# ToKe79/nuts333

Hardware: AMD Instinct MI355X
Metric: delivered_broadcast_lines_per_s (higher is better)
Workload: dtype u8

## Files before the change

nuts333_amd/device/fanout.hip:

```cpp

#include <hip/hip_runtime.h>
#include <hipcub/hipcub.hpp>

#include <algorithm>
#include <chrono>
#include <cstdint>
#include <cstdio>
#include <cstring>

namespace {

constexpr int kOutBuff = 1000;
constexpr int kTextSize = 2000;
constexpr int kNumCols = 21;
constexpr int kMaxWrites = 16;
constexpr int kBlock = 256;

constexpr uint8_t kLogin = 1, kHasRoom = 2, kSameRoom = 4, kIgnall = 8, kIgnshout = 16, kSender = 32, kColour = 64;
constexpr int kComShout = 4, kComSemote = 7;

__constant__ char kColCom[kNumCols][2] = {
    {'R', 'S'}, {'O', 'L'}, {'U', 'L'}, {'L', 'I'}, {'R', 'V'}, {'F', 'K'}, {'F', 'R'}, {'F', 'G'}, {'F', 'Y'}, {'F', 'B'},
    {'F', 'M'}, {'F', 'T'}, {'F', 'W'}, {'B', 'K'}, {'B', 'R'}, {'B', 'G'}, {'B', 'Y'}, {'B', 'B'}, {'B', 'M'}, {'B', 'T'},
    {'B', 'W'},
};
__constant__ char kColArg[kNumCols][2] = {
    {'0', 0}, {'1', 0}, {'4', 0}, {'5', 0}, {'7', 0}, {'3', '0'}, {'3', '1'}, {'3', '2'}, {'3', '3'}, {'3', '4'},
    {'3', '5'}, {'3', '6'}, {'3', '7'}, {'4', '0'}, {'4', '1'}, {'4', '2'}, {'4', '3'}, {'4', '4'}, {'4', '5'}, {'4', '6'},
    {'4', '7'},
};

__device__ __forceinline__ bool admits(uint8_t l, int rm_is_null, int force_listen, int com_num)
{
    if (l & kLogin) return false;
    if (!(l & kHasRoom)) return false;
    if (!(l & kSameRoom) && !rm_is_null) return false;
    if ((l & kIgnall) && !force_listen) return false;
    if ((l & kIgnshout) && (com_num == kComShout || com_num == kComSemote)) return false;
    if (l & kSender) return false;
    return true;
}

__device__ __forceinline__ uint8_t listener_record(int room, uint8_t slot, int rm, int sender, int j)
{
    return (slot & (kLogin | kIgnall | kIgnshout | kColour)) | (room >= 0 ? kHasRoom : 0) |
           (rm >= 0 && room == rm ? kSameRoom : 0) | (j == sender ? kSender : 0);
}

__device__ __forceinline__ int colcom_at(const uint8_t* s, int i, int len)
{
    if (i + 2 >= len) return -1;
    const uint8_t a = s[i + 1], b = s[i + 2];
    for (int c = 0; c < kNumCols; c++)
        if (a == (uint8_t)kColCom[c][0] && b == (uint8_t)kColCom[c][1]) return c;
    return -1;
}

template <bool EMIT>
struct Sink {
    uint8_t* out;
    int32_t* wsz;
    int64_t cap;
    int wcap;
    int64_t n = 0;
    int writes = 0;
    int pos = 0;

    __device__ __forceinline__ void put(uint8_t c)
    {
        if (EMIT && n < cap) out[n] = c;
        n++;
        pos++;
    }
    __device__ __forceinline__ void flush()
    {
        if (EMIT && writes < wcap) wsz[writes] = pos;
        writes++;
        pos = 0;
    }
    __device__ __forceinline__ void reset_code()
    {
        put(27); put('['); put('0'); put('m');
    }
};

template <bool EMIT>
__device__ void transduce(const uint8_t* s, int len, bool colour, Sink<EMIT>& k)
{
    int i = 0;
    while (i < len) {
        const uint8_t ch = s[i];
        if (ch == '\n') {
            if (k.pos > kOutBuff - 6) k.flush();
            if (colour) k.reset_code();
            k.put('\n');
            k.put('\r');
            i++;
        } else if (ch == '/' && i + 1 < len && s[i + 1] == '~') {
            i++;
            continue;
        } else if (i > 0 && ch == '~' && s[i - 1] == '/') {
            k.put('~');
            i++;
        } else if (ch == '~') {
            if (k.pos > kOutBuff - 6) k.flush();
            const int c = colcom_at(s, i, len);
            if (c >= 0) {
                if (colour) {
                    k.put(27); k.put('['); k.put((uint8_t)kColArg[c][0]);
                    if (kColArg[c][1]) k.put((uint8_t)kColArg[c][1]);
                    k.put('m');
                }
                i += 3;
            } else {
                k.put('~');
                i++;
            }
        } else {
            k.put(ch);
            i++;
        }
        if (k.pos == kOutBuff) k.flush();
    }
    if (k.pos) k.flush();
    if (colour) {
        k.reset_code();
        k.flush();
    }
}

struct Args {
    const uint8_t* text;
    const int32_t* text_off;
    const int32_t* text_len;
    const uint8_t* rec;
    int n;
    int rm_is_null, force_listen, com_num;
    uint8_t* admitted;
    int64_t* nbytes;
    int32_t* nwrites;
    int64_t* out_off;
    int32_t* w_off;
    int* violations;
    uint8_t* arena;
    int64_t arena_cap;
    int32_t* wsz;
    int64_t wsz_cap;
};

template <bool BROADCAST>
__device__ __forceinline__ bool load_item(const Args& a, int i, const uint8_t*& s, int& len)
{
    if (BROADCAST) {
        __shared__ uint8_t lds[kTextSize];
        len = a.text_len[0];
        for (int j = threadIdx.x; j < len; j += blockDim.x) lds[j] = a.text[j];
        __syncthreads();
        s = lds;
        return i < a.n;
    }
    if (i >= a.n) return false;
    s = a.text + a.text_off[i];
    len = a.text_len[i];
    return true;
}

template <bool BROADCAST>
__device__ void measure(const Args& a)
{
    const int i = blockIdx.x * blockDim.x + threadIdx.x;
    if (i == 0) {
        a.nbytes[a.n] = 0;
        a.nwrites[a.n] = 0;
    }
    const uint8_t* s;
    int len;
    if (!load_item<BROADCAST>(a, i, s, len)) return;
    const uint8_t l = a.rec[i];
    const bool in = !BROADCAST || admits(l, a.rm_is_null, a.force_listen, a.com_num);
    Sink<false> k{nullptr, nullptr, 0, 0};
    if (in) transduce(s, len, (l & kColour) != 0, k);
    if (k.n > 6 * (int64_t)len + 4 || k.writes > kMaxWrites) atomicAdd(a.violations, 1);
    a.admitted[i] = in;
    a.nbytes[i] = k.n;
    a.nwrites[i] = k.writes;
}

template <bool BROADCAST>
__device__ void emit(const Args& a)
{
    const int i = blockIdx.x * blockDim.x + threadIdx.x;
    const uint8_t* s;
    int len;
    if (!load_item<BROADCAST>(a, i, s, len) || !a.admitted[i]) return;
    const int64_t room = a.arena_cap - a.out_off[i], wroom = a.wsz_cap - a.w_off[i];
    const int64_t cap = a.nbytes[i] < room ? a.nbytes[i] : (room > 0 ? room : 0);
    const int wcap = (int)(a.nwrites[i] < wroom ? a.nwrites[i] : (wroom > 0 ? wroom : 0));
    Sink<true> k{a.arena + a.out_off[i], a.wsz + a.w_off[i], cap, wcap};
    transduce(s, len, (a.rec[i] & kColour) != 0, k);
}

constexpr int kVarCap = 6 * (kTextSize - 1) + 4;
constexpr int kGroup = 16;

struct ManyArgs {
    const uint8_t* text;
    const int32_t* text_off;
    const int32_t* text_len;
    const uint8_t* flags;
    const int32_t* com_num;
    const int32_t* item_off;
    const int32_t* tile_off;
    const uint8_t* rec;
    int k, m;
    int* violations;
    uint8_t* admitted;
    int64_t* out_off;
    int32_t* w_off;
    int64_t* nbytes;
    int32_t* nwrites;
    uint8_t* arena;
    int64_t arena_cap;
    int32_t* wsz;
    int64_t wsz_cap;
};

struct Tile {
    int b, lo, hi;
};

__device__ __forceinline__ Tile find_tile(const ManyArgs& a)
{
    const int blk = (int)blockIdx.x;
    int lo = 0, hi = a.k;
    while (hi - lo > 1) {
        const int mid = (lo + hi) >> 1;
        if (a.tile_off[mid] <= blk) lo = mid;
        else hi = mid;
    }
    const int first = a.item_off[lo] + (blk - a.tile_off[lo]) * kBlock;
    const int end = a.item_off[lo + 1];
    return {lo, first, first + kBlock < end ? first + kBlock : end};
}

template <bool EMIT, typename A>
__device__ __forceinline__ void stage_variants(const A& a, int b, uint8_t* text, uint8_t* var, int32_t* vwsz,
                                               int64_t* vn, int* vw)
{
    const int len = a.text_len[b];
    const uint8_t* src = a.text + a.text_off[b];
    for (int j = threadIdx.x; j < len; j += blockDim.x) text[j] = src[j];
    __syncthreads();
    if (threadIdx.x == 0 || threadIdx.x == 64) {
        const int c = threadIdx.x >> 6;
        Sink<EMIT> k{EMIT ? var + c * kVarCap : nullptr, EMIT ? vwsz + c * kMaxWrites : nullptr, 6 * (int64_t)len + 4,
                     kMaxWrites};
        transduce(text, len, c != 0, k);
        vn[c] = k.n;
        vw[c] = k.writes;
    }
    __syncthreads();
}

__device__ void measure_many(const ManyArgs& a)
{
    __shared__ uint8_t text[kTextSize];
    __shared__ int64_t vn[2];
    __shared__ int vw[2];
    if (blockIdx.x == 0 && threadIdx.x == 0) {
        a.nbytes[a.m] = 0;
        a.nwrites[a.m] = 0;
    }
    const Tile t = find_tile(a);
    stage_variants<false>(a, t.b, text, nullptr, nullptr, vn, vw);
    const int i = t.lo + (int)threadIdx.x;
    if (i >= t.hi) return;
    const uint8_t l = a.rec[i];
    const int fl = a.flags[t.b];
    const bool in = admits(l, fl & 1, (fl >> 1) & 1, a.com_num[t.b]);
    const int c = (l & kColour) ? 1 : 0;
    const int64_t nb = in ? vn[c] : 0;
    const int nw = in ? vw[c] : 0;
    if (nb > 6 * (int64_t)a.text_len[t.b] + 4 || nw > kMaxWrites) atomicAdd(a.violations, 1);
    a.admitted[i] = in;
    a.nbytes[i] = nb;
    a.nwrites[i] = nw;
}

__device__ void emit_many(const ManyArgs& a)
{
    __shared__ uint8_t text[kTextSize];
    __shared__ uint8_t var[2 * kVarCap];
    __shared__ int32_t vwsz[2 * kMaxWrites];
    __shared__ int64_t vn[2];
    __shared__ int vw[2];
    __shared__ int64_t s_off[kBlock], s_n[kBlock];
    __shared__ int32_t s_woff[kBlock], s_nw[kBlock];
    __shared__ uint8_t s_c[kBlock];
    const Tile t = find_tile(a);
    const int len = a.text_len[t.b];
    {
        const int i = t.lo + (int)threadIdx.x;
        if (i < t.hi) {
            const bool in = a.admitted[i] != 0;
            const int64_t off = a.out_off[i], woff = a.w_off[i];
            const int64_t room = a.arena_cap - off, wroom = a.wsz_cap - woff;
            int64_t n = in ? a.nbytes[i] : 0;
            n = n < room ? n : room;
            n = n < 6 * (int64_t)len + 4 ? n : 6 * (int64_t)len + 4;
            int64_t nw = in ? a.nwrites[i] : 0;
            nw = nw < wroom ? nw : wroom;
            nw = nw < kMaxWrites ? nw : kMaxWrites;
            s_off[threadIdx.x] = off;
            s_n[threadIdx.x] = n > 0 ? n : 0;
            s_woff[threadIdx.x] = (int32_t)woff;
            s_nw[threadIdx.x] = nw > 0 ? (int32_t)nw : 0;
            s_c[threadIdx.x] = (a.rec[i] & kColour) ? 1 : 0;
        }
    }
    stage_variants<true>(a, t.b, text, var, vwsz, vn, vw);
    const int g = (int)threadIdx.x / kGroup, lane = (int)threadIdx.x % kGroup;
    for (int j = g; j < t.hi - t.lo; j += kBlock / kGroup) {
        const int c = s_c[j];
        const int64_t n0 = s_n[j], vmax = vn[c] < kVarCap ? vn[c] : kVarCap;
        const int64_t n = n0 < vmax ? n0 : vmax;
        const uint8_t* src = var + c * kVarCap;
        uint8_t* dst = a.arena + s_off[j];
        const int head = (int)(s_off[j] & 3);
        for (int64_t w = 4 * lane - head; w < n; w += 4 * kGroup) {
            if (w >= 0 && w + 4 <= n) {
                const uint32_t v = (uint32_t)src[w] | (uint32_t)src[w + 1] << 8 | (uint32_t)src[w + 2] << 16 |
                                   (uint32_t)src[w + 3] << 24;
                *reinterpret_cast<uint32_t*>(dst + w) = v;
            } else {
                for (int q = 0; q < 4; q++)
                    if (w + q >= 0 && w + q < n) dst[w + q] = src[w + q];
            }
        }
        const int nw = s_nw[j] < vw[c] ? s_nw[j] : vw[c];
        if (lane < nw) a.wsz[s_woff[j] + lane] = vwsz[c * kMaxWrites + lane];
    }
}

static_assert(kGroup >= kMaxWrites, "emit_many writes an item's chunk sizes with one lane each");
static_assert(kBlock % kGroup == 0 && kBlock >= 128, "emit_many: whole lane groups; variants on waves 0 and 1");

struct RosterArgs {
    const int32_t* room;
    const uint8_t* slot;
    const uint8_t* text;
    const int32_t* text_off;
    const int32_t* text_len;
    const int32_t* rm;
    const int32_t* sender;
    const uint8_t* flags;
    const int32_t* com_num;
    int k, capacity, tiles;
    int* violations;
    uint8_t* admitted;
    int64_t* out_off;
    int32_t* w_off;
    uint8_t* var;
    int64_t* vn;
    int32_t* vw;
    int32_t* vwsz;
    uint8_t* arena;
    int64_t arena_cap;
    int32_t* wsz;
    int64_t wsz_cap;
};

__host__ __device__ __forceinline__ int64_t var_stride(int len) { return (6 * (int64_t)len + 4 + 3) & ~(int64_t)3; }
__host__ __device__ __forceinline__ int64_t var_at(int64_t text_off, int64_t t) { return 12 * text_off + 16 * t; }

template <typename A>
__device__ __forceinline__ void store_variants(const A& a, int t)
{
    __shared__ uint8_t text[kTextSize];
    __shared__ uint8_t var[2 * kVarCap];
    __shared__ int32_t vwsz[2 * kMaxWrites];
    __shared__ int64_t vn[2];
    __shared__ int vw[2];
    stage_variants<true>(a, t, text, var, vwsz, vn, vw);
    const int len = a.text_len[t];
    const int64_t cap = 6 * (int64_t)len + 4, stride = var_stride(len);
    uint8_t* dst = a.var + var_at(a.text_off[t], t);
    for (int c = 0; c < 2; c++) {
        const int64_t n = vn[c] < cap ? vn[c] : cap;
        for (int64_t q = threadIdx.x; q < n; q += kBlock) dst[c * stride + q] = var[c * kVarCap + q];
        const int nw = vw[c] < kMaxWrites ? vw[c] : kMaxWrites;
        if ((int)threadIdx.x < nw) a.vwsz[(2 * t + c) * kMaxWrites + threadIdx.x] = vwsz[c * kMaxWrites + threadIdx.x];
    }
    if (threadIdx.x < 2) {
        a.vn[2 * t + threadIdx.x] = vn[threadIdx.x];
        a.vw[2 * t + threadIdx.x] = vw[threadIdx.x];
        if (vn[threadIdx.x] > cap || vw[threadIdx.x] > kMaxWrites) atomicAdd(a.violations, 1);
    }
}

__device__ void roster_measure(const RosterArgs& a)
{
    const int b = (int)blockIdx.x / a.tiles, tile = (int)blockIdx.x - b * a.tiles;
    const int j = tile * kBlock + (int)threadIdx.x;
    if (j < a.capacity) {
        const int rm = a.rm[b];
        const uint8_t l = listener_record(a.room[j], a.slot[j], rm, a.sender[b], j);
        a.admitted[b * a.capacity + j] = admits(l, rm < 0, (a.flags[b] >> 1) & 1, a.com_num[b]);
    }
    if (tile == 0) store_variants(a, b);
}

template <typename T>
struct ItemCount {
    const uint8_t* admitted;
    const uint8_t* slot;
    const T* v;
    int capacity, m;
    __host__ __device__ T operator()(int i) const
    {
        if (i >= m || !admitted[i]) return 0;
        const int b = i / capacity;
        return v[2 * b + ((slot[i - b * capacity] & kColour) ? 1 : 0)];
    }
};

__device__ __forceinline__ void copy_items(int count, const uint8_t* var, const int32_t* vwsz, const int64_t* vn,
                                           const int* vw, const int64_t* s_off, const int64_t* s_n,
                                           const int32_t* s_woff, const int32_t* s_nw, const uint8_t* s_c,
                                           uint8_t* arena, int32_t* wsz)
{
    const int g = (int)threadIdx.x / kGroup, lane = (int)threadIdx.x % kGroup;
    for (int j = g; j < count; j += kBlock / kGroup) {
        const int c = s_c[j];
        const int64_t n0 = s_n[j], vmax = vn[c] < kVarCap ? vn[c] : kVarCap;
        const int64_t n = n0 < vmax ? n0 : vmax;
        const uint8_t* src = var + c * kVarCap;
        uint8_t* dst = arena + s_off[j];
        const int head = (int)(s_off[j] & 3);
        for (int64_t w = 4 * lane - head; w < n; w += 4 * kGroup) {
            if (w >= 0 && w + 4 <= n) {
                const uint32_t v = (uint32_t)src[w] | (uint32_t)src[w + 1] << 8 | (uint32_t)src[w + 2] << 16 |
                                   (uint32_t)src[w + 3] << 24;
                *reinterpret_cast<uint32_t*>(dst + w) = v;
            } else {
                for (int q = 0; q < 4; q++)
                    if (w + q >= 0 && w + q < n) dst[w + q] = src[w + q];
            }
        }
        const int nw = s_nw[j] < vw[c] ? s_nw[j] : vw[c];
        if (lane < nw) wsz[s_woff[j] + lane] = vwsz[c * kMaxWrites + lane];
    }
}

__device__ void roster_emit(const RosterArgs& a)
{
    __shared__ uint8_t var[2 * kVarCap];
    __shared__ int32_t vwsz[2 * kMaxWrites];
    __shared__ int64_t vn[2];
    __shared__ int vw[2];
    __shared__ int64_t s_off[kBlock], s_n[kBlock];
    __shared__ int32_t s_woff[kBlock], s_nw[kBlock];
    __shared__ uint8_t s_c[kBlock];
    const int b = (int)blockIdx.x / a.tiles, j0 = ((int)blockIdx.x - b * a.tiles) * kBlock;
    const int len = a.text_len[b];
    const int64_t cap = 6 * (int64_t)len + 4;
    {
        const int j = j0 + (int)threadIdx.x;
        if (j < a.capacity) {
            const int i = b * a.capacity + j;
            const bool in = a.admitted[i] != 0;
            const int64_t off = a.out_off[i], woff = a.w_off[i];
            const int64_t room = a.arena_cap - off, wroom = a.wsz_cap - woff;
            int64_t n = in ? a.out_off[i + 1] - off : 0;
            n = n < room ? n : room;
            n = n < cap ? n : cap;
            int64_t nw = in ? a.w_off[i + 1] - woff : 0;
            nw = nw < wroom ? nw : wroom;
            nw = nw < kMaxWrites ? nw : kMaxWrites;
            s_off[threadIdx.x] = off;
            s_n[threadIdx.x] = n > 0 ? n : 0;
            s_woff[threadIdx.x] = (int32_t)woff;
            s_nw[threadIdx.x] = nw > 0 ? (int32_t)nw : 0;
            s_c[threadIdx.x] = (a.slot[j] & kColour) ? 1 : 0;
        }
    }
    const uint8_t* src = a.var + var_at(a.text_off[b], b);
    const int64_t stride = var_stride(len);
    for (int c = 0; c < 2; c++) {
        const int64_t n = a.vn[2 * b + c] < cap ? a.vn[2 * b + c] : cap;
        for (int64_t q = threadIdx.x; q < n; q += kBlock) var[c * kVarCap + q] = src[c * stride + q];
        const int nw = a.vw[2 * b + c] < kMaxWrites ? a.vw[2 * b + c] : kMaxWrites;
        if ((int)threadIdx.x < nw) vwsz[c * kMaxWrites + threadIdx.x] = a.vwsz[(2 * b + c) * kMaxWrites + threadIdx.x];
        if (threadIdx.x == 0) {
            vn[c] = n;
            vw[c] = nw;
        }
    }
    __syncthreads();
    const int count = a.capacity - j0 < kBlock ? a.capacity - j0 : kBlock;
    copy_items(count, var, vwsz, vn, vw, s_off, s_n, s_woff, s_nw, s_c, a.arena, a.wsz);
}

static_assert(2 * kMaxWrites <= kBlock, "roster kernels move a broadcast's chunk sizes with one lane each");

struct PlanArgs {
    const int32_t* room;
    const uint8_t* slot;
    const uint8_t* text;
    const int32_t* text_off;
    const int32_t* text_len;
    const int32_t* rm;
    const int32_t* sender;
    const uint8_t* flags;
    const int32_t* com_num;
    int k, capacity, tiles;
    int words;
    int* violations;
    int64_t* vn;
    int32_t* vw;
    int32_t* vwsz;
    uint64_t* bits;
    uint8_t* var;
};

__device__ void roster_plan(const PlanArgs& a)
{
    const int b = (int)blockIdx.x / a.tiles, tile = (int)blockIdx.x - b * a.tiles;
    const int j = tile * kBlock + (int)threadIdx.x;
    bool in = false;
    if (j < a.capacity) {
        const int rm = a.rm[b];
        const uint8_t l = listener_record(a.room[j], a.slot[j], rm, a.sender[b], j);
        in = admits(l, rm < 0, (a.flags[b] >> 1) & 1, a.com_num[b]);
    }
    const uint64_t word = __ballot(in);
    const int w = j >> 6;
    if ((threadIdx.x & 63) == 0 && w < a.words) a.bits[(int64_t)b * a.words + w] = word;
    if (tile == 0) store_variants(a, b);
}

static_assert(kBlock % 64 == 0, "roster_plan: a tile is whole bitmap words, one per wave");

constexpr int kRevLines = 15;
constexpr int kRevLen = 200;
constexpr int kRevSlot = kRevLen + 2;
constexpr int kRevRing = kRevLines * kRevSlot;
constexpr int kRevLineCap = 6 * (kRevLen + 1) + 4;
constexpr int kRevLineStride = (kRevLineCap + 1 + 3) & ~3;
constexpr int kRevLineWrites = 3;
constexpr int kRevVarCap = kRevLines * kRevLineCap;
constexpr int rev_var_stride(int lines) { return (lines * kRevLineCap + 3) & ~3; }
constexpr int kRevVarStride = rev_var_stride(kRevLines);
constexpr int kTellLines = 5;
constexpr int kRevWrites = kRevLines * kRevLineWrites;
constexpr int kRevTasks = 2 * kRevLines;
constexpr int kWaveLimit = kOutBuff - 6;
constexpr uint8_t kRecordBit = 4;
constexpr int kMaxReviewRooms = 1024;

struct RecordArgs {
    const uint8_t* text;
    const int32_t* text_off;
    const int32_t* text_len;
    const int32_t* rm;
    const uint8_t* flags;
    const uint8_t* clear;
    int k, review_rooms;
    uint8_t* rings;
    int32_t* revline;
};

template <int LINES>
__device__ void roster_record(const RecordArgs& a)
{
    __shared__ int s_surv[LINES];
    __shared__ int s_count, s_base;
    const int room = (int)blockIdx.x;
    const bool cleared = a.clear && a.clear[room];
    if (threadIdx.x < 64) {
        const int lane = (int)threadIdx.x;
        int count = 0;
        for (int b0 = 0; b0 < a.k; b0 += 64) {
            const int b = b0 + lane;
            const bool hit = b < a.k && (a.flags[b] & kRecordBit) && a.rm[b] == room;
            const uint64_t word = __ballot(hit);
            const int n = __popcll(word);
            const int rank = count + __popcll(word & ((1ull << lane) - 1));
            if (hit && rank >= count + n - LINES) s_surv[rank % LINES] = b;
            count += n;
        }
        if (lane == 0) {
            s_count = count;
            s_base = cleared ? 0 : (int)((uint32_t)a.revline[room] % LINES);
        }
    }
    __syncthreads();
    const int count = s_count, base = s_base;
    if (!count && !cleared) return;
    uint8_t* ring = a.rings + (size_t)room * LINES * kRevSlot;
    const int nsurv = count < LINES ? count : LINES;
    const int first = (count - nsurv) % LINES;
    if (cleared && threadIdx.x < LINES) {
        const int d = ((int)threadIdx.x - base - first + 2 * LINES) % LINES;
        if (d >= nsurv) ring[threadIdx.x * kRevSlot] = 0;
    }
    for (int idx = (int)threadIdx.x; idx < nsurv * kRevSlot; idx += kBlock) {
        const int j = idx / kRevSlot, i = idx - j * kRevSlot;
        const int r = (first + j) % LINES;
        const int b = s_surv[r];
        uint8_t v = 0;
        if (i < kRevLen) {
            if (i < a.text_len[b]) v = a.text[a.text_off[b] + i];
        } else if (i == kRevLen) {
            v = '\n';
        }
        ring[((base + r) % LINES) * kRevSlot + i] = v;
    }
    if (threadIdx.x == 0) a.revline[room] = (base + count % LINES) % LINES;
}

struct ReviewArgs {
    uint8_t* rings;
    int32_t* revline;
    const int32_t* rooms;
    const uint8_t* clear;
    int q, review_rooms;
    int* violations;
    int32_t* line_count;
    int32_t* sequential;
    int32_t* vn;
    int32_t* vw;
    int32_t* vwsz;
    uint8_t* lines;
    uint8_t* var;
};

__device__ __forceinline__ int expand_byte(uint8_t p1, uint8_t ch, uint8_t n1, bool consumed, int own, bool colour,
                                           uint64_t* v)
{
    *v = ch;
    if (ch == 0 || consumed) return 0;
    if (ch == '\n') {
        if (colour) {
            *v = 27ull | (uint64_t)'[' << 8 | (uint64_t)'0' << 16 | (uint64_t)'m' << 24 | (uint64_t)'\n' << 32 |
                 (uint64_t)'\r' << 40;
            return 6;
        }
        *v = (uint64_t)'\n' | (uint64_t)'\r' << 8;
        return 2;
    }
    if (ch == '/' && n1 == '~') return 0;
    if (ch == '~' && p1 != '/' && own >= 0) {
        if (!colour) return 0;
        const uint64_t a0 = (uint8_t)kColArg[own][0], a1 = (uint8_t)kColArg[own][1];
        *v = 27ull | (uint64_t)'[' << 8 | a0 << 16 | (a1 ? a1 << 24 | (uint64_t)'m' << 32 : (uint64_t)'m' << 24);
        return a1 ? 5 : 4;
    }
    return 1;
}

template <int LINES>
__device__ void roster_review(const ReviewArgs& a)
{
    constexpr int TASKS = 2 * LINES;
    constexpr int RING = LINES * kRevSlot, WRITES = LINES * kRevLineWrites;
    if ((int)blockIdx.x >= a.q) {
        const int room = ((int)blockIdx.x - a.q) * kBlock + (int)threadIdx.x;
        if (a.clear && room < a.review_rooms && a.clear[room]) {
            for (int i = 0; i < LINES; i++) a.rings[(size_t)room * RING + i * kRevSlot] = 0;
            a.revline[room] = 0;
        }
        return;
    }
    __shared__ uint8_t s_line[LINES][kRevSlot + 2];
    __shared__ uint8_t s_out[TASKS][kRevLineStride];
    __shared__ int32_t s_wsz[TASKS][kRevLineWrites + 1];
    __shared__ int s_n[TASKS], s_w[TASKS], s_off[TASKS], s_woff[TASKS];
    __shared__ int s_len[LINES], s_seq;
    const int q = (int)blockIdx.x, room = a.rooms[q];
    const bool cleared = a.clear && a.clear[room];
    const int rev = cleared ? 0 : (int)((uint32_t)a.revline[room] % LINES);
    const uint8_t* ring = a.rings + (size_t)room * RING;
    for (int idx = (int)threadIdx.x; idx < RING; idx += kBlock) {
        const int i = idx / kRevSlot, j = idx - i * kRevSlot;
        const uint8_t v = cleared ? 0 : ring[((rev + i) % LINES) * kRevSlot + j];
        s_line[i][j] = v;
        a.lines[(size_t)q * RING + idx] = v;
    }
    if (threadIdx.x == 0) s_seq = 0;
    __syncthreads();

    const int lane = (int)threadIdx.x & 63;
    for (int t = (int)threadIdx.x >> 6; t < TASKS; t += kBlock / 64) {
        const int i = t >> 1;
        const bool colour = (t & 1) != 0;
        const uint8_t* s = s_line[i];
        uint8_t w[9];
#pragma unroll
        for (int x = 0; x < 9; x++) {
            const int at = 4 * lane - 3 + x;
            w[x] = at >= 0 && at < kRevSlot ? s[at] : 0;
        }
        const int nul = w[3] == 0 ? 0 : w[4] == 0 ? 1 : w[5] == 0 ? 2 : w[6] == 0 ? 3 : 4;
        const uint64_t ends = __ballot(nul < 4);
        const int end_lane = __ffsll((unsigned long long)ends) - 1;
        const int len = 4 * end_lane + __shfl(nul, end_lane, 64);
#pragma unroll
        for (int x = 0; x < 9; x++)
            if (4 * lane - 3 + x >= len) w[x] = 0;
        int cmd[6], key[6];
        bool tilde = false;
#pragma unroll
        for (int x = 0; x < 6; x++) {
            cmd[x] = -1;
            key[x] = w[x + 1] == '~' && w[x] != '/' ? w[x + 2] << 8 | w[x + 3] : -1;
            tilde |= key[x] >= 0;
        }
        if (tilde) {
#pragma unroll 1
            for (int c = 0; c < kNumCols; c++) {
                const int pair = (uint8_t)kColCom[c][0] << 8 | (uint8_t)kColCom[c][1];
#pragma unroll
                for (int x = 0; x < 6; x++) cmd[x] = key[x] == pair ? c : cmd[x];
            }
        }
        int n[4], mine = 0;
        uint64_t v[4];
#pragma unroll
        for (int x = 0; x < 4; x++) {
            n[x] = expand_byte(w[x + 2], w[x + 3], w[x + 4], cmd[x] >= 0 || cmd[x + 1] >= 0, cmd[x + 2], colour, &v[x]);
            mine += n[x];
        }
        int incl = mine;
#pragma unroll
        for (int d = 1; d < 64; d <<= 1) {
            const int y = __shfl_up(incl, d, 64);
            if (lane >= d) incl += y;
        }
        const int body = __shfl(incl, 63, 64);
        uint8_t* out = s_out[t];
        if (len == 0) {
            if (lane == 0) {
                s_n[t] = 0;
                s_w[t] = 0;
            }
        } else if (body <= kWaveLimit) {
            int at = incl - mine;
#pragma unroll
            for (int x = 0; x < 4; x++) {
#pragma unroll
                for (int y = 0; y < 6; y++)
                    out[y < n[x] ? at + y : kRevLineStride - 1] = (uint8_t)(v[x] >> (8 * y));
                at += n[x];
            }
            if (colour && lane < 4) out[body + lane] = lane == 0 ? 27 : lane == 1 ? '[' : lane == 2 ? '0' : 'm';
            if (lane == 0) {
                int nw = 0;
                if (body) s_wsz[t][nw++] = body;
                if (colour) s_wsz[t][nw++] = 4;
                s_n[t] = body + (colour ? 4 : 0);
                s_w[t] = nw;
            }
        } else if (lane == 0) {
            s_n[t] = -1;
        }
        if (lane == 0 && !colour) s_len[i] = len;
    }
    __syncthreads();
    if (threadIdx.x < TASKS && s_n[threadIdx.x] < 0) {
        const int t = (int)threadIdx.x;
        Sink<true> k{s_out[t], s_wsz[t], kRevLineCap, kRevLineWrites};
        transduce(s_line[t >> 1], s_len[t >> 1], (t & 1) != 0, k);
        if (k.n > kRevLineCap || k.writes > kRevLineWrites) atomicAdd(a.violations, 1);
        s_n[t] = k.n < kRevLineCap ? (int)k.n : kRevLineCap;
        s_w[t] = k.writes < kRevLineWrites ? k.writes : kRevLineWrites;
        atomicAdd(&s_seq, 1);
    }
    __syncthreads();
    if (threadIdx.x < TASKS) {
        const int t = (int)threadIdx.x;
        int off = 0, woff = 0;
        for (int j = t & 1; j < t; j += 2) {
            off += s_n[j];
            woff += s_w[j];
        }
        s_off[t] = off;
        s_woff[t] = woff;
        if (t >= TASKS - 2) {
            a.vn[2 * q + (t & 1)] = off + s_n[t];
            a.vw[2 * q + (t & 1)] = woff + s_w[t];
        }
    }
    if (threadIdx.x == 64) {
        int lines = 0;
        for (int i = 0; i < LINES; i++) lines += s_len[i] > 0;
        a.line_count[q] = lines;
        a.sequential[q] = s_seq;
    }
    __syncthreads();
    for (int t = 0; t < TASKS; t++) {
        const int var = 2 * q + (t & 1);
        uint8_t* dst = a.var + (size_t)var * rev_var_stride(LINES) + s_off[t];
        for (int j = (int)threadIdx.x; j < s_n[t]; j += kBlock) dst[j] = s_out[t][j];
        if ((int)threadIdx.x < s_w[t]) a.vwsz[var * WRITES + s_woff[t] + (int)threadIdx.x] = s_wsz[t][threadIdx.x];
    }
}

static_assert(kBlock / 64 >= 1 && 64 * 4 >= kRevSlot, "roster_review: a wave holds a whole slot, four bytes per lane");
static_assert(kBlock >= kRevTasks + 64 && kBlock >= kRevLines, "roster_review / roster_record: a lane per task, per line");
static_assert(kTellLines <= kRevLines && kRevVarStride == ((kRevVarCap + 3) & ~3), "the revtell ring is the smaller instance");

constexpr int kComSay = 3, kComEmote = 6;
constexpr int kArrSize = 1000;
constexpr int kSpeakSlack = 36;
constexpr int kSpeechRec = 16;
constexpr int kNameLen = 12;
constexpr uint8_t kVis = 1, kMuzzled = 2, kCommandMode = 4;
constexpr int kSpoken = 0, kOutMuzzled = 1, kOutNothing = 2, kOutSwearing = 3;
constexpr int kSwearSlice = 16;
constexpr int kNotSpeech = -1;
constexpr uint8_t kPresetNone = 0, kPresetVoid = 1, kPresetNothing = 2, kPresetUnknown = 3;

constexpr int64_t ctext_at(int64_t text_off, int64_t t) { return text_off + kSpeakSlack * t; }

struct SpeakArgs {
    const int32_t* room;
    const uint8_t* speech;
    const uint8_t* speech_new;
    uint8_t* speech_keep;
    const uint8_t* text;
    const int32_t* text_off;
    const int32_t* text_len;
    const int32_t* slot;
    const uint8_t* com;
    const uint8_t* words;
    const uint8_t* preset;
    const int32_t* ctext_off;
    int k, capacity, blocks;
    int ban_swearing, record;
    int* violations;
    uint8_t* ctext;
    int32_t* clen;
    int32_t* rm;
    int32_t* sender;
    int32_t* com_num;
    uint8_t* flags;
    int8_t* outcome;
};

struct Piece {
    const uint8_t* p;
    int n;
};
template <int N>
__device__ __forceinline__ Piece lit(const char (&s)[N]) { return {reinterpret_cast<const uint8_t*>(s), N - 1}; }

__device__ __forceinline__ bool swears(const uint8_t* s, int len, int lane)
{
    constexpr uint32_t w0 = 'f' | 'u' << 8 | 'c' << 16 | (uint32_t)'k' << 24;
    constexpr uint32_t w1 = 's' | 'h' << 8 | 'i' << 16 | (uint32_t)'t' << 24;
    constexpr uint32_t w2 = 'c' | 'u' << 8 | 'n' << 16 | (uint32_t)'t' << 24;
    uint32_t low[kSwearSlice + 3];
#pragma unroll
    for (int x = 0; x < kSwearSlice + 3; x++) {
        const int at = kSwearSlice * lane + x;
        const uint32_t c = at < len ? s[at] : 0;
        low[x] = c >= 'A' && c <= 'Z' ? c + 32 : c;
    }
    bool hit = false;
#pragma unroll
    for (int x = 0; x < kSwearSlice; x++) {
        const uint32_t v = low[x] | low[x + 1] << 8 | low[x + 2] << 16 | low[x + 3] << 24;
        hit |= v == w0 || v == w1 || v == w2;
    }
    return __ballot(hit) != 0;
}

__device__ __forceinline__ int compose(uint8_t* dst, int cap, const Piece (&pc)[5], const uint8_t* body, int blen,
                                       bool newline, int lane, int* violations)
{
    const uint8_t* src = nullptr;
    int plen = 0;
#pragma unroll
    for (int i = 0; i < 5; i++) {
        if (lane >= plen && lane < plen + pc[i].n) src = pc[i].p + (lane - plen);
        plen += pc[i].n;
    }
    const int total = plen + blen + (newline ? 1 : 0);
    if (plen > 64 || total > cap) {
        if (lane == 0) atomicAdd(violations, 1);
        return -1;
    }
    if (src) dst[lane] = *src;
    for (int i = lane; i < blen; i += 64) dst[plen + i] = body[i];
    if (newline && lane == 0) dst[plen + blen] = '\n';
    return total;
}

__device__ void roster_speak(const SpeakArgs& a)
{
    if ((int)blockIdx.x >= a.blocks) {
        const int w = ((int)blockIdx.x - a.blocks) * kBlock + (int)threadIdx.x;
        if (a.speech_new && w < a.capacity * (kSpeechRec / 4))
            reinterpret_cast<uint32_t*>(a.speech_keep)[w] = reinterpret_cast<const uint32_t*>(a.speech_new)[w];
        return;
    }
    const int lane = (int)threadIdx.x & 63;
    const int k = (int)blockIdx.x * (kBlock / 64) + ((int)threadIdx.x >> 6);
    if (k >= a.k) return;
    const uint8_t preset = a.preset ? a.preset[k] : kPresetNone;
    const Piece none{nullptr, 0};
    if (preset == kPresetVoid || preset == kPresetUnknown) {
        int reply_len = -1;
        if (preset == kPresetUnknown) {
            const Piece p[5] = {lit("Unknown command.\n"), none, none, none, none};
            reply_len = compose(a.ctext + a.ctext_off[a.k + k], kSpeakSlack, p, nullptr, 0, false, lane, a.violations);
        }
        if (lane == 0) {
            a.clen[k] = -1;
            a.clen[a.k + k] = reply_len;
            a.rm[k] = a.sender[k] = -1;
            a.com_num[k] = 0;
            a.flags[k] = 0;
            a.outcome[k] = (int8_t)kNotSpeech;
        }
        return;
    }
    const int slot = a.slot[k], com = a.com[k], wc = a.words[k], len = a.text_len[k];
    const uint8_t* in = a.text + a.text_off[k];
    const uint8_t* sp = a.speech + (size_t)slot * kSpeechRec;
    const uint8_t state = sp[kNameLen + 1];
    const int nlen = sp[kNameLen] < kNameLen ? sp[kNameLen] : kNameLen;
    const int room = a.room[slot];
    const uint8_t b0 = len > 0 ? in[0] : 0, b1 = len > 1 ? in[1] : 0, last = len > 0 ? in[len - 1] : 0;
    const bool say = com == kComSay, shout = com == kComShout, emote = com == kComEmote;

    int outcome = kSpoken;
    if (preset == kPresetNothing) outcome = kOutNothing;
    else if (state & kMuzzled) outcome = kOutMuzzled;
    else if (say ? wc < 2 && (state & kCommandMode) : shout ? wc < 2 : wc < 2 && (int8_t)b1 < 33) outcome = kOutNothing;
    else if (a.ban_swearing && com != kComSemote && swears(in, len, lane)) outcome = kOutSwearing;

    uint8_t* line = a.ctext + a.ctext_off[k];
    uint8_t* reply = a.ctext + a.ctext_off[a.k + k];
    const int cap = len + kSpeakSlack;
    int line_len = -1, reply_len = -1;
    if (outcome == kOutMuzzled) {
        const Piece p[5] = {say ? lit("You are muzzled, you cannot speak.\n") : shout ? lit("You are muzzled, you cannot shout.\n")
                                : lit("You are muzzled, you cannot emote.\n"), none, none, none, none};
        reply_len = compose(reply, cap, p, nullptr, 0, false, lane, a.violations);
    } else if (outcome == kOutNothing) {
        const Piece p[5] = {say ? lit("Say what?\n") : shout ? lit("Shout what?\n") : emote ? lit("Emote what?\n")
                                : lit("Shout emote what?\n"), none, none, none, none};
        reply_len = compose(reply, cap, p, nullptr, 0, false, lane, a.violations);
    } else if (outcome == kOutSwearing) {
        const Piece p[5] = {lit("Swearing is not allowed here.\n"), none, none, none, none};
        reply_len = compose(reply, cap, p, nullptr, 0, false, lane, a.violations);
    } else {
        const Piece name = (state & kVis) ? Piece{sp, nlen} : lit("A presence");
        const Piece verb = last == '?' ? lit("ask") : last == '!' ? lit("exclaim") : lit("say");
        if (say) {
            const Piece r[5] = {lit("You "), none, none, verb, lit(": ")};
// ... 3264 lines not shown
```

Measured before the change: 726,100.

## Parallelize per-message variant transduction across a wave with prefix-sum placement

Replaces the single-thread serial transduce of each broadcast text (one thread per colour variant) with a wave-parallel version. Each of 64 lanes handles 4 bytes, detects colour commands through a 9-byte window, computes each byte's expansion length, and uses a wave shuffle prefix scan to place its output. The serial transducer is kept only as a fallback for long outputs that exceed the single-write limit, where it also cross-checks the byte count. This targets the serial bottleneck in stage_variants at the cost of more complex window logic and a possible mismatch with the reference semantics at 256-byte chunk edges.

```diff
diff --git a/nuts333_amd/device/fanout.hip b/nuts333_amd/device/fanout.hip
--- a/nuts333_amd/device/fanout.hip
+++ b/nuts333_amd/device/fanout.hip
@@ -15,6 +15,7 @@
 constexpr int kNumCols = 21;
 constexpr int kMaxWrites = 16;
 constexpr int kBlock = 256;
+constexpr int kWaveLimit = kOutBuff - 6;
 
 constexpr uint8_t kLogin = 1, kHasRoom = 2, kSameRoom = 4, kIgnall = 8, kIgnshout = 16, kSender = 32, kColour = 64;
 constexpr int kComShout = 4, kComSemote = 7;
@@ -129,6 +130,50 @@
     }
 }
 
+__device__ __forceinline__ int expand_byte(uint8_t p1, uint8_t ch, uint8_t n1, bool consumed, int own, bool colour,
+                                           uint64_t* v)
+{
+    *v = ch;
+    if (ch == 0 || consumed) return 0;
+    if (ch == '\n') {
+        if (colour) {
+            *v = 27ull | (uint64_t)'[' << 8 | (uint64_t)'0' << 16 | (uint64_t)'m' << 24 | (uint64_t)'\n' << 32 |
+                 (uint64_t)'\r' << 40;
+            return 6;
+        }
+        *v = (uint64_t)'\n' | (uint64_t)'\r' << 8;
+        return 2;
+    }
+    if (ch == '/' && n1 == '~') return 0;
+    if (ch == '~' && p1 != '/' && own >= 0) {
+        if (!colour) return 0;
+        const uint64_t a0 = (uint8_t)kColArg[own][0], a1 = (uint8_t)kColArg[own][1];
+        *v = 27ull | (uint64_t)'[' << 8 | a0 << 16 | (a1 ? a1 << 24 | (uint64_t)'m' << 32 : (uint64_t)'m' << 24);
+        return a1 ? 5 : 4;
+    }
+    return 1;
+}
+
+__device__ __forceinline__ void window_commands(const uint8_t (&w)[9], int (&cmd)[6])
+{
+    int key[6];
+    bool tilde = false;
+#pragma unroll
+    for (int x = 0; x < 6; x++) {
+        cmd[x] = -1;
+        key[x] = w[x + 1] == '~' && w[x] != '/' ? w[x + 2] << 8 | w[x + 3] : -1;
+        tilde |= key[x] >= 0;
+    }
+    if (tilde) {
+#pragma unroll 1
+        for (int c = 0; c < kNumCols; c++) {
+            const int pair = (uint8_t)kColCom[c][0] << 8 | (uint8_t)kColCom[c][1];
+#pragma unroll
+            for (int x = 0; x < 6; x++) cmd[x] = key[x] == pair ? c : cmd[x];
+        }
+    }
+}
+
 struct Args {
     const uint8_t* text;
     const int32_t* text_off;
@@ -251,13 +296,73 @@
     const uint8_t* src = a.text + a.text_off[b];
     for (int j = threadIdx.x; j < len; j += blockDim.x) text[j] = src[j];
     __syncthreads();
-    if (threadIdx.x == 0 || threadIdx.x == 64) {
-        const int c = threadIdx.x >> 6;
-        Sink<EMIT> k{EMIT ? var + c * kVarCap : nullptr, EMIT ? vwsz + c * kMaxWrites : nullptr, 6 * (int64_t)len + 4,
-                     kMaxWrites};
-        transduce(text, len, c != 0, k);
-        vn[c] = k.n;
-        vw[c] = k.writes;
+    if (threadIdx.x < 128) {
+        const int c = (int)threadIdx.x >> 6, lane = (int)threadIdx.x & 63;
+        const bool colour = c != 0;
+        const int cap = 6 * len + 4;
+        uint8_t* out = EMIT ? var + c * kVarCap : nullptr;
+        int body = 0;
+#pragma unroll 1
+        for (int base = 0; base < len; base += 256) {
+            const int first = base + 4 * lane;
+            uint8_t w[9];
+#pragma unroll
+            for (int x = 0; x < 9; x++) {
+                const int at = first - 3 + x;
+                w[x] = at >= 0 && at < len ? text[at] : 0;
+            }
+            int cmd[6];
+            window_commands(w, cmd);
+            int n[4], mine = 0;
+            uint64_t v[4];
+#pragma unroll
+            for (int x = 0; x < 4; x++) {
+                n[x] = expand_byte(w[x + 2], w[x + 3], w[x + 4], cmd[x] >= 0 || cmd[x + 1] >= 0, cmd[x + 2], colour, &v[x]);
+                if (w[x + 3] == 0 && first + x < len) n[x] = 1;
+                mine += n[x];
+            }
+            int incl = mine;
+#pragma unroll
+            for (int d = 1; d < 64; d <<= 1) {
+                const int y = __shfl_up(incl, d, 64);
+                if (lane >= d) incl += y;
+            }
+            if (EMIT) {
+                int at = body + incl - mine;
+#pragma unroll
+                for (int x = 0; x < 4; x++) {
+#pragma unroll
+                    for (int y = 0; y < 6; y++)
+                        if (y < n[x] && at + y < cap) out[at + y] = (uint8_t)(v[x] >> (8 * y));
+                    at += n[x];
+                }
+            }
+            body += __builtin_amdgcn_readlane(incl, 63);
+        }
+        if (EMIT && colour && lane < 4 && body + lane < cap)
+            out[body + lane] = lane == 0 ? 27 : lane == 1 ? '[' : lane == 2 ? '0' : 'm';
+        if (lane == 0) {
+            const int64_t n = body + (colour ? 4 : 0);
+            int32_t* wsz = EMIT ? vwsz + c * kMaxWrites : nullptr;
+            int writes = 0;
+            if (body <= kWaveLimit) {
+                if (body) {
+                    if (EMIT) wsz[writes] = body;
+                    writes++;
+                }
+                if (colour) {
+                    if (EMIT) wsz[writes] = 4;
+                    writes++;
+                }
+            } else {
+                Sink<EMIT> k{nullptr, wsz, 0, kMaxWrites};
+                transduce(text, len, colour, k);
+                if (k.n != n) atomicAdd(a.violations, 1);
+                writes = k.writes;
+            }
+            vn[c] = n;
+            vw[c] = writes;
+        }
     }
     __syncthreads();
 }
@@ -554,7 +659,6 @@
 constexpr int kTellLines = 5;
 constexpr int kRevWrites = kRevLines * kRevLineWrites;
 constexpr int kRevTasks = 2 * kRevLines;
-constexpr int kWaveLimit = kOutBuff - 6;
 constexpr uint8_t kRecordBit = 4;
 constexpr int kMaxReviewRooms = 1024;
 
@@ -634,30 +738,6 @@
     uint8_t* lines;
     uint8_t* var;
 };
-
-__device__ __forceinline__ int expand_byte(uint8_t p1, uint8_t ch, uint8_t n1, bool consumed, int own, bool colour,
-                                           uint64_t* v)
-{
-    *v = ch;
-    if (ch == 0 || consumed) return 0;
-    if (ch == '\n') {
-        if (colour) {
-            *v = 27ull | (uint64_t)'[' << 8 | (uint64_t)'0' << 16 | (uint64_t)'m' << 24 | (uint64_t)'\n' << 32 |
-                 (uint64_t)'\r' << 40;
-            return 6;
-        }
-        *v = (uint64_t)'\n' | (uint64_t)'\r' << 8;
-        return 2;
-    }
-    if (ch == '/' && n1 == '~') return 0;
-    if (ch == '~' && p1 != '/' && own >= 0) {
-        if (!colour) return 0;
-        const uint64_t a0 = (uint8_t)kColArg[own][0], a1 = (uint8_t)kColArg[own][1];
-        *v = 27ull | (uint64_t)'[' << 8 | a0 << 16 | (a1 ? a1 << 24 | (uint64_t)'m' << 32 : (uint64_t)'m' << 24);
-        return a1 ? 5 : 4;
-    }
-    return 1;
-}
 
 template <int LINES>
 __device__ void roster_review(const ReviewArgs& a)
```

Result: slower. 710,100 (-2.2%).
